# BatsResearch/menghini-neurips23-code

Hardware: AMD Instinct MI355X
Metric: images/sec CLIP ViT-B/16 encode+prompt-step (higher is better)
Workload: dtype f16

## Files before the change

### menghini-neurips23-code_amd/csrc/common.h

```cpp
#pragma once
#include <hip/hip_runtime.h>
#include <stdint.h>
#include <stdio.h>
#include <string.h>

#include "host_common.h"
#include "gemm_plan.h"

typedef _Float16 half_t;
typedef half_t half8 __attribute__((ext_vector_type(8)));
typedef half_t half4 __attribute__((ext_vector_type(4)));
typedef half_t half2v __attribute__((ext_vector_type(2)));
typedef float f32x4 __attribute__((ext_vector_type(4)));

typedef half_t resid_t;

#define AS1 __attribute__((address_space(1)))
#define AS3 __attribute__((address_space(3)))

#define GRIP_CHECK_HIP(expr)                                                                   \
    do {                                                                                       \
        hipError_t _e = (expr);                                                                \
        if (_e != hipSuccess) {                                                                \
            grip_set_error("%s:%d %s -> %s", __FILE__, __LINE__, #expr, hipGetErrorString(_e)); \
// ... 16 lines not shown

__device__ __forceinline__ float wave_sum(float v) {
#define GRIP_DPP_ADD(ctrl) v += __builtin_bit_cast(float, __builtin_amdgcn_update_dpp(0, __builtin_bit_cast(int, v), ctrl, 0xF, 0xF, true))
    GRIP_DPP_ADD(0xB1);
    GRIP_DPP_ADD(0x4E);
    GRIP_DPP_ADD(0x141);
    GRIP_DPP_ADD(0x140);
#undef GRIP_DPP_ADD
    const int b = __builtin_bit_cast(int, v);
    const float r0 = __builtin_bit_cast(float, __builtin_amdgcn_readlane(b, 0)), r1 = __builtin_bit_cast(float, __builtin_amdgcn_readlane(b, 16));
    const float r2 = __builtin_bit_cast(float, __builtin_amdgcn_readlane(b, 32)), r3 = __builtin_bit_cast(float, __builtin_amdgcn_readlane(b, 48));
    return (r0 + r1) + (r2 + r3);
}
__device__ __forceinline__ float row16_sum(float v) {
#define GRIP_DPP_ADD(ctrl) v += __builtin_bit_cast(float, __builtin_amdgcn_update_dpp(0, __builtin_bit_cast(int, v), ctrl, 0xF, 0xF, true))
    GRIP_DPP_ADD(0xB1);
    GRIP_DPP_ADD(0x4E);
    GRIP_DPP_ADD(0x141);
    GRIP_DPP_ADD(0x140);
#undef GRIP_DPP_ADD
    return v;
}

__device__ __forceinline__ f32x4 load4(const float* p, int i) { return ((const f32x4*)p)[i]; }
__device__ __forceinline__ f32x4 load4(const half_t* p, int i) {
    const half4 h = ((const half4*)p)[i];
    return (f32x4){(float)h[0], (float)h[1], (float)h[2], (float)h[3]};
}
__device__ __forceinline__ void store4(float* p, int i, f32x4 v) { ((f32x4*)p)[i] = v; }
__device__ __forceinline__ void store4(half_t* p, int i, f32x4 v) { ((half4*)p)[i] = (half4){(half_t)v[0], (half_t)v[1], (half_t)v[2], (half_t)v[3]}; }
#ifndef GRIP_SPLIT_LO_SCALE
#define GRIP_SPLIT_LO_SCALE 1
#endif
struct SplitRow { half_t* p; };
__device__ __forceinline__ void split_f16x4(f32x4 v, half4& hi, half4& lo) {
#pragma unroll
    for (int e = 0; e < 4; ++e) {
        float x = v[e];
        asm volatile("" : "+v"(x));
        const half_t h = (half_t)x;
        hi[e] = h;
        lo[e] = (half_t)((x - (float)h) * (float)GRIP_SPLIT_LO_SCALE);
    }
}
__device__ __forceinline__ void store4(SplitRow r, int i, f32x4 v) {
    half4 hi, lo;
    split_f16x4(v, hi, lo);
    half_t* o = r.p + (i >> 3) * 64 + (i & 7) * 4;
    *(half4*)o = hi;
    *(half4*)(o + 32) = lo;
}

template <int NV>
__device__ __forceinline__ void ln_normalize(f32x4 (&v)[NV], int lane, int d4, int d, float& mean, float& rstd) {
#pragma clang fp contract(off)
    float s = 0.f;
#pragma unroll
    for (int i = 0; i < NV; ++i)
        if (lane + 64 * i < d4) s += v[i][0] + v[i][1] + v[i][2] + v[i][3];
    mean = wave_sum(s) / (float)d;
    float q = 0.f;
#pragma unroll
    for (int i = 0; i < NV; ++i)
        if (lane + 64 * i < d4) {
            f32x4 c = v[i] - mean;
            q += c[0] * c[0] + c[1] * c[1] + c[2] * c[2] + c[3] * c[3];
// ... 11 lines not shown
    const void* W;
    int M, N, K;
    int variant;
    int64_t m_pad;
    const float* bias;
    const void* resid;
    const void* aux;
    void* out;
    void* out2;
    int ldc;
    float scalar;
    int f32;
    float* stat_part;
    const float* rowstat;
    const float* stat_in;
    int stat_parts;
    const float* colsum;
    int ksplit;
    int64_t split_stride;
    float* coop_scratch;
    int* coop_counter;
    int rot_rows;
    half_t* resid_lo;
    int w_exact;
    int ablate;
};

int launch_gemm(int epi, const GemmArgs& a, hipStream_t s);
int launch_gemm_f32(int epi, const GemmArgs& a, hipStream_t s);
int launch_gemm_split(int epi, const GemmArgs& a, hipStream_t s);
int launch_split_rows(const float* x, void* out, int64_t rows, int K, int64_t ld_in, hipStream_t s, int is_weight = 0, int* overflow_flag = nullptr,
                      int* lo_nonzero_flag = nullptr);
float gemm_split_weight_scale();

int launch_im2col(const void* images, int images_f16, void* out, int out_f32, int B, int R, int patch, int Kpad, hipStream_t s);
int launch_vit_assemble_ln(const float* patch_out, const float* cls, const float* pos, const float* prefix, int P,
                           const float* gamma, const float* beta, void* x, int f32, float* rowstat, int B, int G2, int d, hipStream_t s, half_t* x_lo = nullptr,
                           int per_image = 0);
int launch_vit_deep_insert(const float* deep, void* x, int f32, half_t* x_lo, float* stat_part, float* rowstat, int B, int S, int P, int M, int d, hipStream_t s);
int launch_text_deep_insert(const float* deep, int prefix_classes, void* x, int f32, float* stat_part, float* rowstat, int C, int S, int P, int shared_rows, int M, int d,
                            hipStream_t s);
int launch_ln_stats_finalize(const float* stat_part, int parts, float* rowstat, int M, int d, hipStream_t s);
int launch_ln_fold_weights(const half_t* W, const float* gamma, const float* beta, const float* bias, half_t* Wg, float* colsum, float* bias_out,
                           int N, int K, hipStream_t s);
int launch_layernorm_f16(const void* x, const float* gamma, const float* beta, void* out, int f32, int M, int d, hipStream_t s);
int launch_gather_ln_f16(const void* x, const int32_t* row_index, int row_stride, const float* gamma, const float* beta,
                         void* out, int f32, int n_rows, int d, hipStream_t s);
int launch_text_embed(const int32_t* token_ids, int ld_ids, const float* tok_emb, const float* pos, const float* prefix, int P,
                      int prefix_classes, void* x, int f32, float* rowstat, int C, int T, int d, int vocab, hipStream_t s, int shared_rows = 0);
int launch_transpose(const void* in, void* out, int f32, int rows, int cols, int ld_in, hipStream_t s);

#ifdef __HIPCC__
__device__ __forceinline__ size_t seq_row(int b, int r, int S, int Ps) {
    return r < Ps ? (size_t)r : (size_t)Ps + (size_t)b * (S - Ps) + (r - Ps);
}
#endif

int launch_attention_fwd(const half_t* qkv, half_t* out, int B, int S, int H, int causal, hipStream_t s, int shared_rows = 0);
int launch_attention_row(const half_t* qkv, const half_t* qrows, const int32_t* row_index, half_t* out, int B, int S, int H, int causal, hipStream_t s, int train = 0);
int launch_gather_rows(const half_t* x, const int32_t* row_index, int row_stride, half_t* out, int n_rows, int d, hipStream_t s);
int launch_attention_row_bwd(const half_t* qkv, const half_t* o_rows, const half_t* do_rows, const int32_t* row_index, half_t* dqkv, int B, int S, int H, int causal,
                             hipStream_t s);
int launch_attention_fwd_f32(const float* qkv, float* out, int B, int S, int H, int causal, hipStream_t s, int split_out = 0);
int launch_attention_row_f32(const float* qkv, const float* qrows, const int32_t* row_index, float* out, int B, int S, int H, int causal, hipStream_t s, int split_out = 0);
int launch_gather_rows4(const void* x, const int32_t* row_index, int row_stride, void* out, int n_rows, int d, hipStream_t s);
bool attention_split_supported(int S);
// ... 19 lines not shown
```

### menghini-neurips23-code_amd/csrc/gemm.hip

```cpp
#include <type_traits>

#include "common.h"

#ifndef GRIP_COOP_MODE
#define GRIP_COOP_MODE 2
#endif


#ifndef GRIP_RD0
#define GRIP_RD0 4
#endif
#ifndef GRIP_SETPRIO
#define GRIP_SETPRIO 4
#endif
#ifndef GRIP_SMALL_PRIO
#define GRIP_SMALL_PRIO 0
#endif
#ifndef GRIP_KROT
#define GRIP_KROT 1
#endif

#define BM 128
#define BN 128
#define BK 64
// ... 181 lines not shown
                        if (g.out2) *(half4*)((half_t*)g.out2 + o) = (half4){(half_t)v[0], (half_t)v[1], (half_t)v[2], (half_t)v[3]};
                        v = quick_gelu4(v);
                    }
                    *(half4*)((half_t*)g.out + o) = (half4){(half_t)v[0], (half_t)v[1], (half_t)v[2], (half_t)v[3]};
                } else if constexpr (EPI == EPI_GELUGRAD_F16) {
                    const half4 x = aux[p & 1][it];
                    *(half4*)((half_t*)g.out + o) = (half4){(half_t)(v[0] * quick_gelu_grad((float)x[0])), (half_t)(v[1] * quick_gelu_grad((float)x[1])),
                                                            (half_t)(v[2] * quick_gelu_grad((float)x[2])), (half_t)(v[3] * quick_gelu_grad((float)x[3]))};
                }
            }
        }
        __builtin_amdgcn_wave_barrier();
    }
}

template <int EPI, int ROWFRAGS, int PF = 2, bool PRE = false>
__device__ __forceinline__ void epilogue_rows(const GemmArgs& g, f32x4 (&acc)[ROWFRAGS][4], float* slab, int row0, int col0, int lane,
                                              const float2* pre = nullptr, const f32x4* cb = nullptr) {
    if constexpr (EPI == EPI_BIAS_RESID_STATS) {
        if (g.resid_lo) {
            if (row0 + ROWFRAGS * 16 <= g.M)
                epilogue_rows_impl<EPI, ROWFRAGS, false, PF, PRE, true>(g, acc, slab, row0, col0, lane, pre, cb);
            else
                epilogue_rows_impl<EPI, ROWFRAGS, true, PF, PRE, true>(g, acc, slab, row0, col0, lane, pre, cb);
            return;
        }
    }
    if (row0 + ROWFRAGS * 16 <= g.M)
        epilogue_rows_impl<EPI, ROWFRAGS, false, PF, PRE>(g, acc, slab, row0, col0, lane, pre, cb);
    else
        epilogue_rows_impl<EPI, ROWFRAGS, true, PF, PRE>(g, acc, slab, row0, col0, lane, pre, cb);
}

__device__ __forceinline__ float row8_sum(float v) {
#define GRIP_DPP_ADD(ctrl) v += __builtin_bit_cast(float, __builtin_amdgcn_update_dpp(0, __builtin_bit_cast(int, v), ctrl, 0xF, 0xF, true))
    GRIP_DPP_ADD(0xB1);
    GRIP_DPP_ADD(0x4E);
    GRIP_DPP_ADD(0x141);
#undef GRIP_DPP_ADD
    return v;
}

template <int EPI, bool CHECK, bool PRE, bool HILO = false>
__device__ __forceinline__ void epilogue_rows8_impl(const GemmArgs& g, f32x4 (&acc)[8][4], float* slab, int row0, int col0, int lane, const float2* pre) {
    constexpr bool FOLD = (EPI == EPI_LNFOLD_F16 || EPI == EPI_LNFOLD_GELU_F16);
    constexpr bool RESID = (EPI == EPI_BIAS_RESID_STATS);
    static_assert(FOLD || RESID, "epilogue_rows8: f16-output epilogues of the pool encode only");
    const int frow = lane & 15, fgrp = lane >> 4;
    const int r8 = lane >> 3, c8 = lane & 7;
    const int col = col0 + c8 * 8;
    const int ldc = g.ldc;
    const uint32_t lane_off = (uint32_t)(row0 + r8) * (uint32_t)ldc + (uint32_t)col;
    auto elem_off = [&](int p, int it) -> uint32_t {
        if constexpr (CHECK) {
            int row = row0 + p * 16 + it * 8 + r8;
            row = row < g.M ? row : g.M - 1;
            return (uint32_t)row * (uint32_t)ldc + (uint32_t)col;
        } else {
            return lane_off + (uint32_t)((p * 16 + it * 8) * ldc);
        }
    };
    half8 res[2][2];
    half8 resl[2][HILO ? 2 : 1];
    auto prefetch = [&](int p, int b) {
#pragma unroll
        for (int it = 0; it < 2; ++it) {
// ... 1052 lines not shown
    auto spread = [&]() {
#pragma unroll
        for (int q = 0; q < 12; ++q) {
            __builtin_amdgcn_sched_group_barrier(0x008, 2, 0);
            __builtin_amdgcn_sched_group_barrier(0x100, 1, 0);
        }
    };

    const int nk = g.K / BK;
    auto tile_rot = [&](int tile) {
        int tm, tn;
        tile_coords(tile, tm, tn);
        return k_rot(tn, tiles_n, nk);
    };
    auto ks = [&](int k, int rot) { return k + rot < nk ? k + rot : k + rot - nk; };
    const half_t* src_cur = tile_src(t);
    int rot_cur = tile_rot(t);
    stage(0, src_cur, ks(0, rot_cur));
    stage(1, src_cur, ks(1, rot_cur));
    wait_vmcnt<GI>();
    __builtin_amdgcn_s_barrier();
    int par = 0;
    for (;;) {
        int tm, tn;
        tile_coords(t, tm, tn);
        const int m0 = tm * BMT, n0 = tn * BNT;
        const int t_next = t + per_xcd;
        const bool has_next = t_next < xcount;
        const half_t* src_next = has_next ? tile_src(t_next) : src_cur;
        const int rot_next = has_next ? tile_rot(t_next) : 0;
        if constexpr (EPI == EPI_BIAS_F16 || EPI == EPI_BIAS_GELU_F16 || EPI == EPI_BIAS_RESID || EPI == EPI_BIAS_RESID_STATS) {
#pragma unroll
            for (int j = 0; j < 4; ++j) {
                const f32x4 b = *(const f32x4*)(g.bias + n0 + wc * 64 + (EMODE == 2 ? (lane >> 4) * 16 + j * 4 : j * 16 + (lane >> 4) * 4));
#pragma unroll
                for (int i = 0; i < 8; ++i) acc[i][j] = b;
            }
        } else {
#pragma unroll
            for (int i = 0; i < 8; ++i)
#pragma unroll
                for (int j = 0; j < 4; ++j) acc[i][j] = (f32x4){0.f, 0.f, 0.f, 0.f};
        }
        float2 pre[2];
        if constexpr (EPI == EPI_LNFOLD_F16 || EPI == EPI_LNFOLD_GELU_F16) {
#pragma unroll
            for (int h = 0; h < 2; ++h) {
                int r = m0 + wr * 128 + h * 64 + lane;
                r = r < g.M ? r : g.M - 1;
                pre[h] = ((const float2*)g.rowstat)[r];
            }
        }
        load_frags(0, par, 0);
        for (int kt = 0; kt < nk; ++kt) {
            const int buf = (par + kt) & 1;
            load_frags(1, buf, 1);
            constexpr bool PRIO0 = (GRIP_SETPRIO & 1) && GRIP_SETPRIO < 4;
            constexpr bool PRIO1 = ((GRIP_SETPRIO & 2) && GRIP_SETPRIO < 4) || (GRIP_SETPRIO == 4 && (EPI == EPI_LNFOLD_F16 || EPI == EPI_LNFOLD_GELU_F16));
            if constexpr (PRIO0) __builtin_amdgcn_s_setprio(1);
            mfma_set(0);
            spread();
            if constexpr (PRIO0) __builtin_amdgcn_s_setprio(0);
            asm volatile("s_waitcnt lgkmcnt(0)" ::: "memory");
            wait_vmcnt<0>();
            __builtin_amdgcn_s_barrier();
            if constexpr (PRIO1) __builtin_amdgcn_s_setprio(1);
            if constexpr (SD) {
                const half_t* sp = kt + 2 < nk ? src_cur + (size_t)ks(kt + 2, rot_cur) * BK : (has_next ? src_next + (size_t)ks(kt + 2 - nk, rot_next) * BK : src_cur);
                half_t* dst = lds2 + buf * STAGE + r0 * BK;
                const half_t* st = lds2 + (buf ^ 1) * STAGE;
                constexpr int RD0 = GRIP_RD0;
#pragma unroll
                for (int q = 0; q < 16; ++q) {
#pragma unroll
                    for (int h = 0; h < 2; ++h) {
                        const int mi = (2 * q + h) >> 2, mj = (2 * q + h) & 3;
                        acc[mi][mj] = __builtin_amdgcn_mfma_f32_16x16x32_f16(fb[1][mj], fa[1][mi], acc[mi][mj], 0, 0, 0);
                    }
                    if (q >= RD0 && q < RD0 + 4) fb[0][q - RD0] = *(const half8*)(st + b_off[0] + (q - RD0) * BJ * BK);
                    else if (q >= RD0 + 4 && q < RD0 + 12) fa[0][q - RD0 - 4] = *(const half8*)(st + a_off[0] + (q - RD0 - 4) * 16 * BK);
                    if (q < GI)
                        __builtin_amdgcn_global_load_lds((const AS1 void*)((const char*)(sp + (size_t)q * 8 * K) + lane_off[(q >> 1) & 1]), (AS3 void*)(dst + q * 8 * BK), 16, 0, 0);
                    __builtin_amdgcn_sched_group_barrier(0x008, 2, 0);
                    if (q >= RD0 && q < RD0 + 12) __builtin_amdgcn_sched_group_barrier(0x100, 1, 0);
                    if (q < GI) __builtin_amdgcn_sched_group_barrier(0x010, 1, 0);
                }
            } else {
                if (kt + 2 < nk) stage(buf, src_cur, ks(kt + 2, rot_cur));
                else if (has_next) stage(buf, src_next, ks(kt + 2 - nk, rot_next));
                if (kt + 1 < nk) load_frags(0, buf ^ 1, 0);
                mfma_set(1);
                spread();
            }
            if constexpr (PRIO1) __builtin_amdgcn_s_setprio(0);
        }
        if constexpr (EMODE == 4)
            epilogue_rows8h<EPI, true>(g, acc, (half_t*)slab, m0 + wr * 128, n0 + wc * 64, lane, pre);
        else if constexpr (EMODE == 2)
            epilogue_direct<EPI, (EPI == EPI_LNFOLD_F16 || EPI == EPI_LNFOLD_GELU_F16)>(g, acc, m0 + wr * 128, n0 + wc * 64, lane, pre);
        else if constexpr (EMODE == 1)
            epilogue_rows8<EPI, (EPI == EPI_LNFOLD_F16 || EPI == EPI_LNFOLD_GELU_F16)>(g, acc, slab, m0 + wr * 128, n0 + wc * 64, lane, pre);
        else
            epilogue_rows<EPI, 8, 1, (EPI == EPI_LNFOLD_F16 || EPI == EPI_LNFOLD_GELU_F16)>(g, acc, slab, m0 + wr * 128, n0 + wc * 64, lane, pre);
        if (!has_next) break;
        par = (par + nk) & 1;
        t = t_next;
        src_cur = src_next;
        rot_cur = rot_next;
    }
}

#include <deque>
#include <vector>
namespace {
constexpr int PROF_RING = 4096, PROF_EPIS = 144;
struct ProfRec { int epi; double flops; hipEvent_t a, b; };
bool g_prof = false;
std::deque<ProfRec> g_recs;
std::vector<hipEvent_t> g_pool;
int64_t g_launches[PROF_EPIS];
double g_ms[PROF_EPIS], g_flops[PROF_EPIS];
hipEvent_t prof_event() {
    if (!g_pool.empty()) { hipEvent_t e = g_pool.back(); g_pool.pop_back(); return e; }
    hipEvent_t e = nullptr;
    if (hipEventCreate(&e) != hipSuccess) return nullptr;
    return e;
}
void prof_drain(size_t keep) {
    while (g_recs.size() > keep) {
// ... 129 lines not shown
#ifdef GRIP_ABLATE
    a.ablate = g_ablate;
#endif
    return with_epi(p.epi, [&](auto e) {
        constexpr int E = decltype(e)::value;
        if constexpr (E == EPI_LNFOLD_F16 || E == EPI_LNFOLD_GELU_F16) {
            if (p.sd) return launch_planned<gemm_k64p_kernel<E, (E == EPI_LNFOLD_F16 ? 4 : 2), true>>(p, a, s, p.colgroup);
            switch (p.emode) {
                case 4: return launch_planned<gemm_k64p_kernel<E, 4>>(p, a, s, p.colgroup);
                case 2: return launch_planned<gemm_k64p_kernel<E, 2>>(p, a, s, p.colgroup);
                case 1: return launch_planned<gemm_k64p_kernel<E, 1>>(p, a, s, p.colgroup);
            }
        } else if constexpr (E == EPI_BIAS_RESID_STATS) {
            if (p.sd) return launch_planned<gemm_k64p_kernel<E, 1, true>>(p, a, s, p.colgroup);
            if (p.emode == 1) return launch_planned<gemm_k64p_kernel<E, 1>>(p, a, s, p.colgroup);
        }
        return launch_planned<gemm_k64p_kernel<E>>(p, a, s, p.colgroup);
    });
}

static int gemm_cu_count(int* n_cu) {
    static int n_cu_dev = 0;
    if (!n_cu_dev) {
        int dev = 0;
        GRIP_CHECK_HIP(hipGetDevice(&dev));
        GRIP_CHECK_HIP(hipDeviceGetAttribute(&n_cu_dev, hipDeviceAttributeMultiprocessorCount, dev));
        n_cu_dev &= ~7;
        GRIP_REQUIRE(n_cu_dev >= 8, "gemm: device reports %d CUs", n_cu_dev);
    }
    *n_cu = (grip_cu_budget() > 0 && grip_cu_budget() < n_cu_dev) ? (grip_cu_budget() & ~7) : n_cu_dev;
    return GRIP_OK;
}

static int launch_gemm_impl(int epi, const GemmArgs& a_in, hipStream_t s, int* chosen) {
    GemmShape g{};
    g.epi = epi; g.M = a_in.M; g.N = a_in.N; g.K = a_in.K; g.ldc = a_in.ldc; g.m_pad = a_in.m_pad;
    g.variant = a_in.variant; g.ksplit = a_in.ksplit; g.f32 = a_in.f32; g.rot_rows = a_in.rot_rows;
    g.stat_parts = a_in.stat_parts; g.split_stride = a_in.split_stride;
    g.stat_part = a_in.stat_part; g.stat_in = a_in.stat_in; g.rowstat = a_in.rowstat; g.out2 = a_in.out2; g.coop = a_in.coop_scratch && a_in.coop_counter;
    if (!a_in.f32) {
        const int rc = gemm_cu_count(&g.n_cu);
        if (rc) return rc;
    }
    const GemmPlan p = gemm_plan(g, gemm_tuning());
    if (p.status) {
        grip_set_error("%s", p.msg);
        return p.status;
    }
    *chosen = p.variant;
    GemmArgs a = a_in;
    a.rot_rows = p.rot_rows;
    if (p.finalize_stats) {
        const int rc = launch_ln_stats_finalize(a.stat_in, a.stat_parts, const_cast<float*>(a.rowstat), a.M, a.K, s);
        if (rc) return rc;
        a.stat_parts = 0;
    }
    switch (p.family) {
        case GEMM_SPLIT: return launch_gemm_split(epi, a, s);
        case GEMM_F32: return launch_gemm_f32(epi, a, s);
        case GEMM_TWO_STAGE: return launch_two_stage(p, a, s);
        case GEMM_RING: return launch_ring(p, a, s);
        case GEMM_RINGW: return launch_ringw(p, a, s);
        case GEMM_BIG: return launch_big(p, a, s);
        case GEMM_K64: return launch_k64(p, a, s);
        case GEMM_K64P: return launch_k64p(p, a, s);
    }
// ... 3 lines not shown
```

### menghini-neurips23-code_amd/csrc/gemm_split.hip

```cpp
#include <math.h>

#include "common.h"

#if defined(__HIP_DEVICE_COMPILE__) && !defined(__gfx950__)
#error "gemm_split.hip relies on gfx950 MFMA semantics (unflushed f16 subnormal inputs); build with --offload-arch=gfx950 only"
#endif

#define SPL_BM 256
#define SPL_BN 128
#define SPL_ROWB 128
#define SPL_STAGE_B ((SPL_BM + SPL_BN) * SPL_ROWB)
#define SPL_NST 3
#ifndef SPL_PIPE
#define SPL_PIPE 1
#endif
#define SPL_LO_INV (1.0f / (float)GRIP_SPLIT_LO_SCALE)

__device__ __forceinline__ float quick_gelu_exact_s(float x) { return x * __builtin_amdgcn_rcpf(1.0f + __builtin_amdgcn_exp2f(-1.702f * 1.4426950408889634f * x)); }


#if GRIP_SPLIT_LO_SCALE != 1
template <int EPI>
__global__ __launch_bounds__(512, 2) void gemm_split_kernel(GemmArgs g, int tiles_m, int tiles_n) {
    extern __shared__ __attribute__((aligned(16))) char lds[];

    const int nwg = tiles_m * tiles_n;
    int bid = blockIdx.x;
    {
        const int q = nwg >> 3, r = nwg & 7, xcd = bid & 7, idx = bid >> 3;
        bid = (xcd < r ? xcd * (q + 1) : r * (q + 1) + (xcd - r) * q) + idx;
    }
    const int tm = bid / tiles_n, tn = bid - tm * tiles_n;
    const int m0 = tm * SPL_BM, n0 = tn * SPL_BN;

    const int tid = threadIdx.x;
    const int lane = tid & 63;
    const int wave = __builtin_amdgcn_readfirstlane(tid >> 6);
    const int wr = wave >> 1, wc = wave & 1;

    const int srow = lane >> 3;
    const int schunk = (lane & 7) ^ srow;
    const size_t pitch = (size_t)g.K * 4;
    const char* a_src = (const char*)g.A + (size_t)(m0 + wave * 32) * pitch;
    const char* w_src = (const char*)g.W + (size_t)(n0 + wave * 16) * pitch;
    const uint32_t lane_off = (uint32_t)srow * (uint32_t)pitch + (uint32_t)(schunk * 16);
    auto stage = [&](int slot, int kt) {
        char* abase = lds + slot * SPL_STAGE_B + wave * 32 * SPL_ROWB;
        char* bbase = lds + slot * SPL_STAGE_B + SPL_BM * SPL_ROWB + wave * 16 * SPL_ROWB;
        const char* as = a_src + (size_t)kt * SPL_ROWB;
        const char* ws = w_src + (size_t)kt * SPL_ROWB;
#pragma unroll
// ... 115 lines not shown
#endif
    asm volatile("s_waitcnt vmcnt(0)" ::: "memory");

    constexpr bool HAS_BIAS = (EPI == EPI_BIAS_F16 || EPI == EPI_BIAS_GELU_F16 || EPI == EPI_BIAS_RESID);
    const int row0 = m0 + wr * 64 + frow, col0 = n0 + wc * 64 + fgrp * 4;
#pragma unroll
    for (int j = 0; j < 4; ++j) {
        f32x4 b = {0.f, 0.f, 0.f, 0.f};
        if constexpr (HAS_BIAS) b = *(const f32x4*)(g.bias + col0 + j * 16);
#pragma unroll
        for (int i = 0; i < 4; ++i) {
            const int row = row0 + i * 16;
            if (row >= g.M) continue;
            const int col = col0 + j * 16;
            f32x4 v = acc[i][j] + cor[i][j] * SPL_LO_INV + b;
            if constexpr (EPI == EPI_BIAS_RESID) v += *(const f32x4*)((const float*)g.resid + (size_t)row * g.ldc + col);
            if constexpr (EPI == EPI_BIAS_GELU_F16) {
                v = (f32x4){quick_gelu_exact_s(v[0]), quick_gelu_exact_s(v[1]), quick_gelu_exact_s(v[2]), quick_gelu_exact_s(v[3])};
                store4(SplitRow{(half_t*)g.out + (size_t)row * 2 * g.ldc}, col >> 2, v);
            } else {
                *(f32x4*)((float*)g.out + (size_t)row * g.ldc + col) = v;
            }
        }
    }
}

#endif


#if GRIP_SPLIT_LO_SCALE == 1
#define SP1_BM 256
#define SP1_BN 256
#define SP1_STAGE_B ((SP1_BM + SP1_BN) * SPL_ROWB)
#define SP1_W_SCALE 256.0f
template <int EPI, bool WLO>
__global__ __launch_bounds__(512, 2) void gemm_split1_kernel(GemmArgs g, int tiles_m, int tiles_n) {
    constexpr int FI = 4, FJ = 8;
    extern __shared__ __attribute__((aligned(16))) char lds[];
    const int nwg = tiles_m * tiles_n;
    int bid = blockIdx.x;
    {
        const int q = nwg >> 3, r = nwg & 7, xcd = bid & 7, idx = bid >> 3;
        bid = (xcd < r ? xcd * (q + 1) : r * (q + 1) + (xcd - r) * q) + idx;
    }
    const int tm = bid / tiles_n, tn = bid - tm * tiles_n;
    const int m0 = tm * SP1_BM, n0 = tn * SP1_BN;
    const int tid = threadIdx.x;
    const int lane = tid & 63;
    const int wave = __builtin_amdgcn_readfirstlane(tid >> 6);
    const int wr = wave >> 1, wc = wave & 1;

    const int srow = lane >> 3;
    const int schunk = (lane & 7) ^ srow;
    const size_t pitch = (size_t)g.K * 4;
    const char* a_src = (const char*)g.A + (size_t)(m0 + wave * 32) * pitch;
    const char* w_src = (const char*)g.W + (size_t)(n0 + wave * 32) * pitch;
    const uint32_t lane_off = (uint32_t)srow * (uint32_t)pitch + (uint32_t)(schunk * 16);

    const int frow = lane & 15, fgrp = lane >> 4;
    const int swz_hi = (fgrp ^ (lane & 7)) * 16, swz_lo = ((4 + fgrp) ^ (lane & 7)) * 16;
    const int a_row = (wr * FI * 16 + frow) * SPL_ROWB;
    const int b_row = SP1_BM * SPL_ROWB + (wc * FJ * 16 + frow) * SPL_ROWB;

    f32x4 acc[FI][FJ];
#pragma unroll
    for (int i = 0; i < FI; ++i)
#pragma unroll
        for (int j = 0; j < FJ; ++j) acc[i][j] = (f32x4){0.f, 0.f, 0.f, 0.f};

    const int nk = g.K / 32;
    int ks_stage = (int)(((int64_t)tn * nk) / tiles_n);
    auto next_slice = [&](int k) { return k + 1 == nk ? 0 : k + 1; };
    {
        char* abase = lds + wave * 32 * SPL_ROWB;
        char* bbase = lds + SP1_BM * SPL_ROWB + wave * 32 * SPL_ROWB;
        const char* as = a_src + (size_t)ks_stage * SPL_ROWB;
        const char* ws = w_src + (size_t)ks_stage * SPL_ROWB;
#pragma unroll
        for (int pc = 0; pc < 4; ++pc) {
            __builtin_amdgcn_global_load_lds((const AS1 void*)(as + (size_t)pc * 8 * pitch + lane_off), (AS3 void*)(abase + pc * 8 * SPL_ROWB), 16, 0, 0);
            __builtin_amdgcn_global_load_lds((const AS1 void*)(ws + (size_t)pc * 8 * pitch + lane_off), (AS3 void*)(bbase + pc * 8 * SPL_ROWB), 16, 0, 0);
        }
        ks_stage = next_slice(ks_stage);
    }
    for (int kt = 0; kt < nk; ++kt) {
        asm volatile("s_waitcnt vmcnt(0)" ::: "memory");
        __builtin_amdgcn_s_barrier();
        const char* st = lds + (kt & 1) * SP1_STAGE_B;
        half8 ah[FI], al[FI], wh[FJ], wl[FJ];
        wh[0] = *(const half8*)(st + b_row + swz_hi);
#pragma unroll
        for (int i = 0; i < FI; ++i) ah[i] = *(const half8*)(st + a_row + i * 16 * SPL_ROWB + swz_hi);
#pragma unroll
        for (int j = 1; j < FJ; ++j) wh[j] = *(const half8*)(st + b_row + j * 16 * SPL_ROWB + swz_hi);
        __builtin_amdgcn_sched_barrier(0);
        char* abase = lds + ((kt + 1) & 1) * SP1_STAGE_B + wave * 32 * SPL_ROWB;
        char* bbase = lds + ((kt + 1) & 1) * SP1_STAGE_B + SP1_BM * SPL_ROWB + wave * 32 * SPL_ROWB;
        const char* as = a_src + (size_t)ks_stage * SPL_ROWB;
        const char* ws = w_src + (size_t)ks_stage * SPL_ROWB;
        ks_stage = next_slice(ks_stage);
        constexpr int NQ = WLO ? 96 : 64, PIECE_EVERY = NQ / 8, LO_READS = WLO ? 12 : FI;
#pragma unroll
        for (int q = 0; q < NQ; ++q) {
            const int pass = q >> 5, j = ((q & 31) / FI), i = q % FI;
            if (pass == 0) acc[i][j] = __builtin_amdgcn_mfma_f32_16x16x32_f16(wh[j], ah[i], acc[i][j], 0, 0, 0);
            else if (WLO && pass == 1) acc[i][j] = __builtin_amdgcn_mfma_f32_16x16x32_f16(wl[j], ah[i], acc[i][j], 0, 0, 0);
            else acc[i][j] = __builtin_amdgcn_mfma_f32_16x16x32_f16(wh[j], al[i], acc[i][j], 0, 0, 0);
            if (q < 2 * LO_READS && !(q & 1)) {
                const int r = (q >> 1) + (WLO ? 0 : FJ);
                if (r < FJ) wl[r] = *(const half8*)(st + b_row + r * 16 * SPL_ROWB + swz_lo);
                else al[r - FJ] = *(const half8*)(st + a_row + (r - FJ) * 16 * SPL_ROWB + swz_lo);
                __builtin_amdgcn_sched_barrier(0);
            }
            if (q % PIECE_EVERY == PIECE_EVERY - 1) {
                const int pc = q / PIECE_EVERY;
                if (pc < 4) __builtin_amdgcn_global_load_lds((const AS1 void*)(as + (size_t)pc * 8 * pitch + lane_off), (AS3 void*)(abase + pc * 8 * SPL_ROWB), 16, 0, 0);
                else __builtin_amdgcn_global_load_lds((const AS1 void*)(ws + (size_t)(pc - 4) * 8 * pitch + lane_off), (AS3 void*)(bbase + (pc - 4) * 8 * SPL_ROWB), 16, 0, 0);
                __builtin_amdgcn_sched_barrier(0);
            }
        }
        __builtin_amdgcn_sched_barrier(0);
    }
    asm volatile("s_waitcnt vmcnt(0)" ::: "memory");

    constexpr bool HAS_BIAS = (EPI == EPI_BIAS_F16 || EPI == EPI_BIAS_GELU_F16 || EPI == EPI_BIAS_RESID);
    const int row0 = m0 + wr * FI * 16 + frow, col0 = n0 + wc * FJ * 16 + fgrp * 4;
#pragma unroll
    for (int j = 0; j < FJ; ++j) {
        f32x4 b = {0.f, 0.f, 0.f, 0.f};
        if constexpr (HAS_BIAS) b = *(const f32x4*)(g.bias + col0 + j * 16);
#pragma unroll
        for (int i = 0; i < FI; ++i) {
            const int row = row0 + i * 16;
            if (row >= g.M) continue;
            const int col = col0 + j * 16;
            f32x4 v = acc[i][j] * (1.0f / SP1_W_SCALE) + b;
            if constexpr (EPI == EPI_BIAS_RESID) v += *(const f32x4*)((const float*)g.resid + (size_t)row * g.ldc + col);
            if constexpr (EPI == EPI_BIAS_GELU_F16) {
                v = (f32x4){quick_gelu_exact_s(v[0]), quick_gelu_exact_s(v[1]), quick_gelu_exact_s(v[2]), quick_gelu_exact_s(v[3])};
                store4(SplitRow{(half_t*)g.out + (size_t)row * 2 * g.ldc}, col >> 2, v);
            } else {
                *(f32x4*)((float*)g.out + (size_t)row * g.ldc + col) = v;
            }
        }
    }
}
#endif

__global__ __launch_bounds__(256) void split_rows_kernel(const float* __restrict__ x, half_t* __restrict__ out, int64_t rows, int K, int64_t ld_in, float scale,
                                                         int* __restrict__ overflow, int* __restrict__ lo_nonzero) {
    const int64_t i = (int64_t)blockIdx.x * 256 + threadIdx.x;
    const int k4 = K >> 2;
    if (i >= rows * k4) return;
    const int64_t r = i / k4;
    const int c = (int)(i - r * k4) * 4;
    const f32x4 v = *(const f32x4*)(x + r * ld_in + c) * scale;
    if (overflow) {
        const float m = fmaxf(fmaxf(fabsf(v.x), fabsf(v.y)), fmaxf(fabsf(v.z), fabsf(v.w)));
        if (!(m < 65520.0f)) *overflow = 1;
    }
    if (lo_nonzero) {
        const bool exact = (float)(half_t)v.x == v.x && (float)(half_t)v.y == v.y && (float)(half_t)v.z == v.z && (float)(half_t)v.w == v.w;
        if (!exact) *lo_nonzero = 1;
    }
    store4(SplitRow{out + r * 2 * (int64_t)K}, c >> 2, v);
}

float gemm_split_weight_scale() {
#if GRIP_SPLIT_LO_SCALE == 1
    return SP1_W_SCALE;
#else
    return 1.0f;
#endif
}

int launch_split_rows(const float* x, void* out, int64_t rows, int K, int64_t ld_in, hipStream_t s, int is_weight, int* overflow_flag, int* lo_nonzero_flag) {
    GRIP_REQUIRE(K % 32 == 0 && rows > 0 && ld_in >= K && ld_in % 4 == 0, "split_rows: need K %% 32 == 0 (rows=%lld K=%d ld=%lld)", (long long)rows, K, (long long)ld_in);
    const int64_t n = rows * (K / 4);
    hipLaunchKernelGGL(split_rows_kernel, dim3((unsigned)((n + 255) / 256)), dim3(256), 0, s, x, (half_t*)out, rows, K, ld_in, is_weight ? gemm_split_weight_scale() : 1.0f,
                       overflow_flag, lo_nonzero_flag);
    GRIP_CHECK_HIP(hipGetLastError());
    return GRIP_OK;
}

static int g_last_wlo = -1;
int gemm_split_last_wlo() { return g_last_wlo; }

int launch_gemm_split(int epi, const GemmArgs& a, hipStream_t s) {
    GRIP_REQUIRE(a.K % 64 == 0 && a.M > 0, "gemm_split: need K %% 64 == 0 (M=%d N=%d K=%d)", a.M, a.N, a.K);
    GRIP_REQUIRE(a.ldc % 32 == 0, "gemm_split: ldc %% 32 != 0");
    GRIP_REQUIRE((int64_t)a.K * 4 * 8 < ((int64_t)1 << 31), "gemm_split: K too large for 32-bit lane offsets");
#if GRIP_SPLIT_LO_SCALE == 1
    constexpr int BM = SP1_BM, BN = SP1_BN;
    constexpr size_t lds = (size_t)2 * SP1_STAGE_B;
#define GRIP_SPLIT_KERNEL(E, WLO) gemm_split1_kernel<E, WLO>
#else
    constexpr int BM = SPL_BM, BN = SPL_BN;
    constexpr size_t lds = (size_t)SPL_NST * SPL_STAGE_B;
#define GRIP_SPLIT_KERNEL(E, WLO) gemm_split_kernel<E>
#endif
    GRIP_REQUIRE(a.N % BN == 0, "gemm_split: need N %% %d == 0 (N=%d)", BN, a.N);
    static const bool force_wlo = getenv("GRIP_SPLIT_WLO") && atoi(getenv("GRIP_SPLIT_WLO")) == 1;
    const bool wlo = !a.w_exact || force_wlo;
    g_last_wlo = wlo;
    const int tiles_m = (a.M + BM - 1) / BM, tiles_n = a.N / BN;
    GRIP_REQUIRE(a.m_pad >= (int64_t)tiles_m * BM, "gemm_split: A must be allocated up to the 256-row tile (M=%d m_pad=%lld)", a.M, (long long)a.m_pad);
    dim3 grid(tiles_m * tiles_n), block(512);
#define GRIP_GEMM_LAUNCH(E, WLO)                                                                                            \
    {                                                                                                                       \
        static bool configured = false;                                                                                     \
        if (!configured) {                                                                                                  \
            GRIP_CHECK_HIP(hipFuncSetAttribute((const void*)GRIP_SPLIT_KERNEL(E, WLO), hipFuncAttributeMaxDynamicSharedMemorySize, (int)lds)); \
            configured = true;                                                                                              \
        }                                                                                                                   \
        hipLaunchKernelGGL((GRIP_SPLIT_KERNEL(E, WLO)), grid, block, lds, s, a, tiles_m, tiles_n);                          \
    }
#define GRIP_GEMM_CASE(E)                                                                                                   \
    case E:                                                                                                                 \
        if (wlo) GRIP_GEMM_LAUNCH(E, true) else GRIP_GEMM_LAUNCH(E, false)                                                  \
        break;
    switch (epi) {
        GRIP_GEMM_CASE(EPI_F32)
        GRIP_GEMM_CASE(EPI_BIAS_F16)
        GRIP_GEMM_CASE(EPI_BIAS_GELU_F16)
        GRIP_GEMM_CASE(EPI_BIAS_RESID)
        default: GRIP_REQUIRE(false, "gemm_split: epilogue %d is not part of the split-f16 (inference) path", epi);
    }
#undef GRIP_GEMM_CASE
#undef GRIP_GEMM_LAUNCH
#undef GRIP_SPLIT_KERNEL
    GRIP_CHECK_HIP(hipGetLastError());
    return GRIP_OK;
}
```

### menghini-neurips23-code_amd/csrc/tower.hip

```cpp
#include <stdarg.h>
#include <stdlib.h>

#include <map>
#include <string>
#include <vector>

#include "common.h"

static thread_local char g_err[512] = "";
void grip_set_error(const char* fmt, ...) {
    va_list ap;
    va_start(ap, fmt);
    vsnprintf(g_err, sizeof(g_err), fmt, ap);
    va_end(ap);
}
extern "C" const char* grip_last_error(void) { return g_err; }
extern "C" int grip_abi_version(void) { return GRIP_ABI_VERSION; }

static int g_cu_budget = 0;
int grip_cu_budget() { return g_cu_budget; }
extern "C" int grip_set_cu_budget(int n_cus) {
    GRIP_REQUIRE(n_cus >= 0 && (n_cus == 0 || n_cus >= 8), "set_cu_budget: %d (0 = all, else at least 8)", n_cus);
    g_cu_budget = n_cus;
    return GRIP_OK;
// ... 329 lines not shown
    GRIP_REQUIRE(t, "tower_finalize: null handle");
    hipStream_t s = (hipStream_t)stream;
    const int d = t->D.width;
    int rc;
    const int f = t->f32;
    if (!f)
        for (const LayerW& w : t->L.layer) {
            if ((rc = launch_transpose(t->wop(w.in_w), t->wop(w.in_wT), f, 3 * d, d, d, s))) return rc;
            if ((rc = launch_transpose(t->wop(w.out_w), t->wop(w.out_wT), f, d, d, d, s))) return rc;
            if ((rc = launch_transpose(t->wop(w.fc_w), t->wop(w.fc_wT), f, 4 * d, d, d, s))) return rc;
            if ((rc = launch_transpose(t->wop(w.proj_w), t->wop(w.proj_wT), f, d, 4 * d, 4 * d, s))) return rc;
        }
    if (!f)
        for (const LayerW& w : t->L.layer) {
            float* F = t->w32;
            if ((rc = launch_ln_fold_weights(t->w16 + w.in_w, F + w.ln1_g, F + w.ln1_b, F + w.in_b, t->w16 + w.in_wG, F + w.in_cs, F + w.in_bb, 3 * d, d, s))) return rc;
            if ((rc = launch_ln_fold_weights(t->w16 + w.fc_w, F + w.ln2_g, F + w.ln2_b, F + w.fc_b, t->w16 + w.fc_wG, F + w.fc_cs, F + w.fc_bb, 4 * d, d, s))) return rc;
        }
    if (t->split) {
        int* flag = nullptr;
        GRIP_CHECK_HIP(hipMalloc((void**)&flag, 2 * sizeof(int)));
        hipError_t e = hipMemsetAsync(flag, 0, 2 * sizeof(int), s);
        rc = e == hipSuccess ? GRIP_OK : GRIP_ERR_HIP;
        for (const LayerW& w : t->L.layer) {
            if (rc) break;
            if ((rc = launch_split_rows((const float*)t->wop(w.in_w), t->wop(w.in_wS), 3 * d, d, d, s, 1, flag, flag + 1))) break;
            if ((rc = launch_split_rows((const float*)t->wop(w.out_w), t->wop(w.out_wS), d, d, d, s, 1, flag, flag + 1))) break;
            if ((rc = launch_split_rows((const float*)t->wop(w.fc_w), t->wop(w.fc_wS), 4 * d, d, d, s, 1, flag, flag + 1))) break;
            if ((rc = launch_split_rows((const float*)t->wop(w.proj_w), t->wop(w.proj_wS), d, 4 * d, 4 * d, s, 1, flag, flag + 1))) break;
        }
        int flags[2] = {0, 0};
        if (!rc && (hipMemcpyAsync(flags, flag, 2 * sizeof(int), hipMemcpyDeviceToHost, s) != hipSuccess || hipStreamSynchronize(s) != hipSuccess)) rc = GRIP_ERR_HIP;
        const int over = flags[0];
        t->w_exact = flags[1] == 0;
        (void)hipFree(flag);
        if (rc == GRIP_ERR_HIP) { grip_set_error("tower_finalize: HIP error while splitting the weights"); return rc; }
        if (rc) return rc;
        GRIP_REQUIRE(!over, "tower_finalize: a block weight times %g leaves the f16 range (or is not finite): split-f16 towers (precision 2) need |w| < %g",
                     (double)gemm_split_weight_scale(), 65504.0 / (double)gemm_split_weight_scale());
    }
    if ((rc = launch_transpose(t->wop(t->L.proj), t->wop(t->L.projT), f, d, t->D.embed_dim, t->D.embed_dim, s))) return rc;
    t->finalized = true;
    return GRIP_OK;
}

extern "C" int grip_workspace_bytes(const grip_tower* t, int batch, int n_prefix, int seq_len, int train, size_t* bytes) {
    GRIP_REQUIRE(t && bytes, "workspace_bytes: null pointer");
    try {
        Workspace w;
        int rc = carve(t, batch, n_prefix, train, nullptr, w, seq_len);
        if (rc) return rc;
        *bytes = w.bytes;
        if (t->D.kind == 1 && n_prefix > 0 && !t->f32) {
            Workspace ws;
            rc = carve(t, batch, n_prefix, train, nullptr, ws, seq_len, 1);
            if (rc) return rc;
            if (ws.bytes > *bytes) *bytes = ws.bytes;
        }
        return GRIP_OK;
    } catch (...) { grip_set_error("workspace_bytes: exception"); return GRIP_ERR_ARG; }
}

#define RUN(expr) do { int _rc = (expr); if (_rc) return _rc; } while (0)

static int run_blocks(grip_tower* t, Workspace& w, resid_t* x0, int causal, const int32_t* read_rows, hipStream_t s, resid_t** x_final, bool* compact) {
    const int d = t->D.width, H = t->D.heads, f = t->f32;
    const int gf = t->split ? 2 : f;
    const float* F = t->w32;
    resid_t* x = x0;
    const int parts = d / 64;
// ... 295 lines not shown
    a.A = A; a.W = W; a.M = M; a.N = N; a.K = K; a.m_pad = m_pad; a.bias = bias; a.resid = resid; a.out = out; a.out2 = out2; a.ldc = N;
    a.stat_part = stat_part; a.rowstat = rowstat; a.colsum = colsum;
    return launch_gemm(epi, a, (hipStream_t)stream);
}
extern "C" int grip_debug_gemm_train(int epi, const void* A, const void* W, int M, int N, int K, const float* bias, const void* resid, void* out, void* out2,
                                     float* stat_part, float* rowstat, const float* colsum, const float* stat_in, int stat_parts, int ksplit,
                                     float* coop_scratch, int* coop_counter, int m_pad, void* stream) {
    GemmArgs a{};
    a.rot_rows = 1;
    a.A = A; a.W = W; a.M = M; a.N = N; a.K = K; a.m_pad = m_pad; a.bias = bias; a.resid = resid; a.out = out; a.out2 = out2; a.ldc = N;
    a.stat_part = stat_part; a.rowstat = rowstat; a.colsum = colsum; a.stat_in = stat_in; a.stat_parts = stat_parts;
    a.ksplit = ksplit; a.coop_scratch = coop_scratch; a.coop_counter = coop_counter;
    return launch_gemm(epi, a, (hipStream_t)stream);
}
extern "C" int grip_debug_coop_split(int M, int N, int K) { return gemm_pick_coop_split(M, N, K); }
extern "C" int grip_debug_ln_fold(const void* W, const float* gamma, const float* beta, const float* bias, void* Wg, float* colsum, float* bias_out,
                                  int N, int K, const float* stat_part, int parts, float* rowstat, int M, int d, void* stream) {
    int rc = W ? launch_ln_fold_weights((const half_t*)W, gamma, beta, bias, (half_t*)Wg, colsum, bias_out, N, K, (hipStream_t)stream) : GRIP_OK;
    if (rc || !stat_part) return rc;
    return launch_ln_stats_finalize(stat_part, parts, rowstat, M, d, (hipStream_t)stream);
}
extern "C" int grip_debug_gemm_split(int epi, const float* A, const float* W, int M, int N, int K, const float* bias, const float* resid, void* out,
                                     void* a_split, void* w_split, int m_pad, void* stream) {
    hipStream_t s = (hipStream_t)stream;
    RUN(launch_split_rows(A, a_split, m_pad, K, K, s));
    int* flag = nullptr;
    GRIP_CHECK_HIP(hipMalloc((void**)&flag, sizeof(int)));
    int inexact = 1;
    int rc = hipMemsetAsync(flag, 0, sizeof(int), s) == hipSuccess ? launch_split_rows(W, w_split, N, K, K, s, 1, nullptr, flag) : GRIP_ERR_HIP;
    if (!rc && (hipMemcpyAsync(&inexact, flag, sizeof(int), hipMemcpyDeviceToHost, s) != hipSuccess || hipStreamSynchronize(s) != hipSuccess)) rc = GRIP_ERR_HIP;
    (void)hipFree(flag);
    if (rc) return rc;
    GemmArgs a{};
    a.w_exact = !inexact;
    a.f32 = 2; a.A = a_split; a.W = w_split; a.M = M; a.N = N; a.K = K; a.m_pad = m_pad; a.bias = bias; a.resid = resid; a.out = out; a.ldc = N;
    return launch_gemm(epi, a, s);
}
int gemm_split_last_wlo();
extern "C" int grip_debug_split_last_wlo(void) { return gemm_split_last_wlo(); }
extern "C" int grip_debug_split_rows(const float* x, void* out, int64_t rows, int K, void* stream) {
    return launch_split_rows(x, out, rows, K, K, (hipStream_t)stream);
}
extern "C" int grip_debug_attention_split(const void* qkv, void* out, int B, int S, int H, int causal, int mfma, void* stream) {
    if (mfma) return launch_attention_fwd_split((const float*)qkv, out, B, S, H, causal, (hipStream_t)stream);
    return launch_attention_fwd_f32((const float*)qkv, (float*)out, B, S, H, causal, (hipStream_t)stream, 1);
}
extern "C" int grip_debug_attention_exact(const void* qkv, void* out, int B, int S, int H, int causal, void* stream) {
    return launch_attention_fwd_f32((const float*)qkv, (float*)out, B, S, H, causal, (hipStream_t)stream);
}
extern "C" int grip_debug_attention(const void* qkv, void* out, int B, int S, int H, int causal, void* stream) {
    return launch_attention_fwd((const half_t*)qkv, (half_t*)out, B, S, H, causal, (hipStream_t)stream);
}
extern "C" int grip_debug_attention_shared(const void* qkv, void* out, int B, int S, int H, int shared_rows, void* stream) {
    return launch_attention_fwd((const half_t*)qkv, (half_t*)out, B, S, H, 1, (hipStream_t)stream, shared_rows);
}
extern "C" int grip_debug_attention_row(const void* qkv, const void* qrows, const int32_t* row_index, void* out, int B, int S, int H, int causal, int train,
                                        void* stream) {
    return launch_attention_row((const half_t*)qkv, (const half_t*)qrows, row_index, (half_t*)out, B, S, H, causal, (hipStream_t)stream, train);
}
extern "C" int grip_debug_attention_row_exact(const void* qkv, const void* qrows, const int32_t* row_index, void* out, int B, int S, int H, int causal,
                                              int split_out, void* stream) {
    return launch_attention_row_f32((const float*)qkv, (const float*)qrows, row_index, (float*)out, B, S, H, causal, (hipStream_t)stream, split_out);
}
extern "C" int grip_debug_layernorm(const float* x, const float* gamma, const float* beta, void* out, int M, int d, void* stream) {
    return launch_layernorm_f16_from_f32(x, gamma, beta, (half_t*)out, M, d, (hipStream_t)stream);
}
extern "C" int grip_debug_ln_bwd_add(const void* x, const float* dln, int parts, int64_t part_stride, const float* gamma, float* dx, void* dxh, int M, int d,
                                     void* stream) {
    return launch_ln_bwd_add((const resid_t*)x, dln, parts, part_stride, gamma, dx, (half_t*)dxh, M, d, (hipStream_t)stream);
// ... 252 lines not shown
```

Before: 20320.

## Route exact-weight split GEMMs through the k64p kernel with duplicated hi weights

When the split-f16 weights have no low part (w_exact), the weight hi half is copied into the lo slot at finalize time. The GEMM then runs as an ordinary f16 GEMM over doubled K, so hi*A_hi + hi*A_lo come out as one dot product, using the tuned k64p kernel with a new split epilogue that handles scaling, residual add and GELU. This drops the dedicated two-pass split1 kernel for this case and trades it for the general planned kernel, at the cost of reading the duplicated weights. Whether it runs depends on the workload's precision mode using the split path.

After: 20750 (median of 6 runs). +2.1%, better.

```diff
diff --git a/menghini-neurips23-code_amd/csrc/common.h b/menghini-neurips23-code_amd/csrc/common.h
--- a/menghini-neurips23-code_amd/csrc/common.h
+++ b/menghini-neurips23-code_amd/csrc/common.h
@@ -72,6 +72,8 @@
 #ifndef GRIP_SPLIT_LO_SCALE
 #define GRIP_SPLIT_LO_SCALE 1
 #endif
+#define SP1_W_SCALE 256.0f
+__device__ __forceinline__ float quick_gelu_exact_s(float x) { return x * __builtin_amdgcn_rcpf(1.0f + __builtin_amdgcn_exp2f(-1.702f * 1.4426950408889634f * x)); }
 struct SplitRow { half_t* p; };
 __device__ __forceinline__ void split_f16x4(f32x4 v, half4& hi, half4& lo) {
 #pragma unroll
@@ -149,6 +151,9 @@
 int launch_split_rows(const float* x, void* out, int64_t rows, int K, int64_t ld_in, hipStream_t s, int is_weight = 0, int* overflow_flag = nullptr,
                       int* lo_nonzero_flag = nullptr);
 float gemm_split_weight_scale();
+bool gemm_split_dup_weights();
+int launch_split_dup_weights(const void* src, void* dst, int64_t rows, int K, hipStream_t s);
+int launch_gemm_split_k64p(int epi, const GemmArgs& a, hipStream_t s);
 
 int launch_im2col(const void* images, int images_f16, void* out, int out_f32, int B, int R, int patch, int Kpad, hipStream_t s);
 int launch_vit_assemble_ln(const float* patch_out, const float* cls, const float* pos, const float* prefix, int P,
diff --git a/menghini-neurips23-code_amd/csrc/gemm.hip b/menghini-neurips23-code_amd/csrc/gemm.hip
--- a/menghini-neurips23-code_amd/csrc/gemm.hip
+++ b/menghini-neurips23-code_amd/csrc/gemm.hip
@@ -237,6 +237,65 @@
         epilogue_rows_impl<EPI, ROWFRAGS, true, PF, PRE>(g, acc, slab, row0, col0, lane, pre, cb);
 }
 
+template <int EPI, bool CHECK>
+__device__ __forceinline__ void epilogue_rows_split_impl(const GemmArgs& g, f32x4 (&acc)[8][4], float* slab, int row0, int col0, int lane) {
+    static_assert(EPI == EPI_F32 || EPI == EPI_BIAS_F16 || EPI == EPI_BIAS_GELU_F16 || EPI == EPI_BIAS_RESID, "epilogue_rows_split: the split tier's four epilogues");
+    constexpr bool RESID = (EPI == EPI_BIAS_RESID);
+    const int frow = lane & 15, fgrp = lane >> 4;
+    const int rr = lane >> 4, cc = (lane & 15) * 4;
+    const int col = col0 + cc;
+    const int ldc = g.ldc;
+    const uint32_t lane_off = (uint32_t)(row0 + rr) * (uint32_t)ldc + (uint32_t)col;
+    auto elem_off = [&](int p, int it) -> uint32_t {
+        if constexpr (CHECK) {
+            int row = row0 + p * 16 + it * 4 + rr;
+            row = row < g.M ? row : g.M - 1;
+            return (uint32_t)row * (uint32_t)ldc + (uint32_t)col;
+        } else {
+            return lane_off + (uint32_t)((p * 16 + it * 4) * ldc);
+        }
+    };
+    f32x4 res[2][RESID ? 4 : 1];
+    auto prefetch = [&](int p, int b) {
+#pragma unroll
+        for (int it = 0; it < 4; ++it) res[b][RESID ? it : 0] = *(const f32x4*)((const float*)g.resid + elem_off(p, it));
+    };
+    if constexpr (RESID) prefetch(0, 0);
+#pragma unroll
+    for (int p = 0; p < 8; ++p) {
+#pragma unroll
+        for (int j = 0; j < 4; ++j) *(f32x4*)(slab + slab_off<1>(frow, j * 4 + fgrp)) = acc[p][j] * (1.0f / SP1_W_SCALE);
+        if constexpr (RESID)
+            if (p + 1 < 8) prefetch(p + 1, (p + 1) & 1);
+        __builtin_amdgcn_wave_barrier();
+#pragma unroll
+        for (int it = 0; it < 4; ++it) {
+            const int rl = it * 4 + rr;
+            f32x4 v = *(const f32x4*)(slab + slab_off<1>(rl, lane & 15));
+            const int row = row0 + p * 16 + rl;
+            const uint32_t o = elem_off(p, it);
+            if constexpr (RESID) v += res[p & 1][it];
+            if (!CHECK || row < g.M) {
+                if constexpr (EPI == EPI_BIAS_GELU_F16) {
+                    v = (f32x4){quick_gelu_exact_s(v[0]), quick_gelu_exact_s(v[1]), quick_gelu_exact_s(v[2]), quick_gelu_exact_s(v[3])};
+                    store4(SplitRow{(half_t*)g.out + 2 * (size_t)(o - (uint32_t)col)}, col >> 2, v);
+                } else {
+                    *(f32x4*)((float*)g.out + o) = v;
+                }
+            }
+        }
+        __builtin_amdgcn_wave_barrier();
+    }
+}
+
+template <int EPI>
+__device__ __forceinline__ void epilogue_rows_split(const GemmArgs& g, f32x4 (&acc)[8][4], float* slab, int row0, int col0, int lane) {
+    if (row0 + 128 <= g.M)
+        epilogue_rows_split_impl<EPI, false>(g, acc, slab, row0, col0, lane);
+    else
+        epilogue_rows_split_impl<EPI, true>(g, acc, slab, row0, col0, lane);
+}
+
 __device__ __forceinline__ float row8_sum(float v) {
 #define GRIP_DPP_ADD(ctrl) v += __builtin_bit_cast(float, __builtin_amdgcn_update_dpp(0, __builtin_bit_cast(int, v), ctrl, 0xF, 0xF, true))
     GRIP_DPP_ADD(0xB1);
@@ -1355,7 +1414,8 @@
         if constexpr (EPI == EPI_BIAS_F16 || EPI == EPI_BIAS_GELU_F16 || EPI == EPI_BIAS_RESID || EPI == EPI_BIAS_RESID_STATS) {
 #pragma unroll
             for (int j = 0; j < 4; ++j) {
-                const f32x4 b = *(const f32x4*)(g.bias + n0 + wc * 64 + (EMODE == 2 ? (lane >> 4) * 16 + j * 4 : j * 16 + (lane >> 4) * 4));
+                f32x4 b = *(const f32x4*)(g.bias + n0 + wc * 64 + (EMODE == 2 ? (lane >> 4) * 16 + j * 4 : j * 16 + (lane >> 4) * 4));
+                if constexpr (EMODE == 3) b *= SP1_W_SCALE;
 #pragma unroll
                 for (int i = 0; i < 8; ++i) acc[i][j] = b;
             }
@@ -1417,7 +1477,9 @@
             }
             if constexpr (PRIO1) __builtin_amdgcn_s_setprio(0);
         }
-        if constexpr (EMODE == 4)
+        if constexpr (EMODE == 3)
+            epilogue_rows_split<EPI>(g, acc, slab, m0 + wr * 128, n0 + wc * 64, lane);
+        else if constexpr (EMODE == 4)
             epilogue_rows8h<EPI, true>(g, acc, (half_t*)slab, m0 + wr * 128, n0 + wc * 64, lane, pre);
         else if constexpr (EMODE == 2)
             epilogue_direct<EPI, (EPI == EPI_LNFOLD_F16 || EPI == EPI_LNFOLD_GELU_F16)>(g, acc, m0 + wr * 128, n0 + wc * 64, lane, pre);
@@ -1613,6 +1675,27 @@
     return GRIP_OK;
 }
 
+int launch_gemm_split_k64p(int epi, const GemmArgs& a_in, hipStream_t s) {
+    GemmShape g{};
+    g.epi = epi; g.M = a_in.M; g.N = a_in.N; g.K = 2 * a_in.K; g.ldc = a_in.ldc; g.m_pad = a_in.m_pad; g.variant = 6;
+    const int rc = gemm_cu_count(&g.n_cu);
+    if (rc) return rc;
+    const GemmPlan p = gemm_plan(g, gemm_tuning());
+    if (p.status) {
+        grip_set_error("%s", p.msg);
+        return p.status;
+    }
+    GemmArgs a = a_in;
+    a.K = g.K;
+    switch (epi) {
+        case EPI_F32: return launch_planned<gemm_k64p_kernel<EPI_F32, 3, true>>(p, a, s, p.colgroup);
+        case EPI_BIAS_F16: return launch_planned<gemm_k64p_kernel<EPI_BIAS_F16, 3, true>>(p, a, s, p.colgroup);
+        case EPI_BIAS_GELU_F16: return launch_planned<gemm_k64p_kernel<EPI_BIAS_GELU_F16, 3, true>>(p, a, s, p.colgroup);
+        case EPI_BIAS_RESID: return launch_planned<gemm_k64p_kernel<EPI_BIAS_RESID, 3, true>>(p, a, s, p.colgroup);
+    }
+    GRIP_REQUIRE(false, "gemm_split: epilogue %d is not part of the split-f16 (inference) path", epi);
+}
+
 static int launch_gemm_impl(int epi, const GemmArgs& a_in, hipStream_t s, int* chosen) {
     GemmShape g{};
     g.epi = epi; g.M = a_in.M; g.N = a_in.N; g.K = a_in.K; g.ldc = a_in.ldc; g.m_pad = a_in.m_pad;
diff --git a/menghini-neurips23-code_amd/csrc/gemm_split.hip b/menghini-neurips23-code_amd/csrc/gemm_split.hip
--- a/menghini-neurips23-code_amd/csrc/gemm_split.hip
+++ b/menghini-neurips23-code_amd/csrc/gemm_split.hip
@@ -15,8 +15,6 @@
 #define SPL_PIPE 1
 #endif
 #define SPL_LO_INV (1.0f / (float)GRIP_SPLIT_LO_SCALE)
-
-__device__ __forceinline__ float quick_gelu_exact_s(float x) { return x * __builtin_amdgcn_rcpf(1.0f + __builtin_amdgcn_exp2f(-1.702f * 1.4426950408889634f * x)); }
 
 
 #if GRIP_SPLIT_LO_SCALE != 1
@@ -198,8 +196,7 @@
 #define SP1_BM 256
 #define SP1_BN 256
 #define SP1_STAGE_B ((SP1_BM + SP1_BN) * SPL_ROWB)
-#define SP1_W_SCALE 256.0f
-template <int EPI, bool WLO>
+template <int EPI>
 __global__ __launch_bounds__(512, 2) void gemm_split1_kernel(GemmArgs g, int tiles_m, int tiles_n) {
     constexpr int FI = 4, FJ = 8;
     extern __shared__ __attribute__((aligned(16))) char lds[];
@@ -265,15 +262,15 @@
         const char* as = a_src + (size_t)ks_stage * SPL_ROWB;
         const char* ws = w_src + (size_t)ks_stage * SPL_ROWB;
         ks_stage = next_slice(ks_stage);
-        constexpr int NQ = WLO ? 96 : 64, PIECE_EVERY = NQ / 8, LO_READS = WLO ? 12 : FI;
+        constexpr int NQ = 96, PIECE_EVERY = NQ / 8, LO_READS = 12;
 #pragma unroll
         for (int q = 0; q < NQ; ++q) {
             const int pass = q >> 5, j = ((q & 31) / FI), i = q % FI;
             if (pass == 0) acc[i][j] = __builtin_amdgcn_mfma_f32_16x16x32_f16(wh[j], ah[i], acc[i][j], 0, 0, 0);
-            else if (WLO && pass == 1) acc[i][j] = __builtin_amdgcn_mfma_f32_16x16x32_f16(wl[j], ah[i], acc[i][j], 0, 0, 0);
+            else if (pass == 1) acc[i][j] = __builtin_amdgcn_mfma_f32_16x16x32_f16(wl[j], ah[i], acc[i][j], 0, 0, 0);
             else acc[i][j] = __builtin_amdgcn_mfma_f32_16x16x32_f16(wh[j], al[i], acc[i][j], 0, 0, 0);
             if (q < 2 * LO_READS && !(q & 1)) {
-                const int r = (q >> 1) + (WLO ? 0 : FJ);
+                const int r = q >> 1;
                 if (r < FJ) wl[r] = *(const half8*)(st + b_row + r * 16 * SPL_ROWB + swz_lo);
                 else al[r - FJ] = *(const half8*)(st + a_row + (r - FJ) * 16 * SPL_ROWB + swz_lo);
                 __builtin_amdgcn_sched_barrier(0);
@@ -332,6 +329,32 @@
     store4(SplitRow{out + r * 2 * (int64_t)K}, c >> 2, v);
 }
 
+__global__ __launch_bounds__(256) void split_dup_weights_kernel(const half_t* src, half_t* dst, int64_t n) {
+    const int64_t i = (int64_t)blockIdx.x * 256 + threadIdx.x;
+    if (i >= n) return;
+    const int64_t o = (i >> 2) * 64 + (i & 3) * 8;
+    const half8 v = *(const half8*)(src + o);
+    *(half8*)(dst + o) = v;
+    *(half8*)(dst + o + 32) = v;
+}
+
+int launch_split_dup_weights(const void* src, void* dst, int64_t rows, int K, hipStream_t s) {
+    GRIP_REQUIRE(K % 32 == 0 && rows > 0, "split_dup_weights: need K %% 32 == 0 (rows=%lld K=%d)", (long long)rows, K);
+    const int64_t n = rows * (K / 8);
+    hipLaunchKernelGGL(split_dup_weights_kernel, dim3((unsigned)((n + 255) / 256)), dim3(256), 0, s, (const half_t*)src, (half_t*)dst, n);
+    GRIP_CHECK_HIP(hipGetLastError());
+    return GRIP_OK;
+}
+
+bool gemm_split_dup_weights() {
+#if GRIP_SPLIT_LO_SCALE == 1
+    static const bool force_wlo = getenv("GRIP_SPLIT_WLO") && atoi(getenv("GRIP_SPLIT_WLO")) == 1;
+    return !force_wlo;
+#else
+    return false;
+#endif
+}
+
 float gemm_split_weight_scale() {
 #if GRIP_SPLIT_LO_SCALE == 1
     return SP1_W_SCALE;
@@ -359,31 +382,35 @@
 #if GRIP_SPLIT_LO_SCALE == 1
     constexpr int BM = SP1_BM, BN = SP1_BN;
     constexpr size_t lds = (size_t)2 * SP1_STAGE_B;
-#define GRIP_SPLIT_KERNEL(E, WLO) gemm_split1_kernel<E, WLO>
+#define GRIP_SPLIT_KERNEL(E) gemm_split1_kernel<E>
 #else
     constexpr int BM = SPL_BM, BN = SPL_BN;
     constexpr size_t lds = (size_t)SPL_NST * SPL_STAGE_B;
-#define GRIP_SPLIT_KERNEL(E, WLO) gemm_split_kernel<E>
+#define GRIP_SPLIT_KERNEL(E) gemm_split_kernel<E>
 #endif
     GRIP_REQUIRE(a.N % BN == 0, "gemm_split: need N %% %d == 0 (N=%d)", BN, a.N);
-    static const bool force_wlo = getenv("GRIP_SPLIT_WLO") && atoi(getenv("GRIP_SPLIT_WLO")) == 1;
-    const bool wlo = !a.w_exact || force_wlo;
+    const bool wlo = !a.w_exact;
     g_last_wlo = wlo;
+#if GRIP_SPLIT_LO_SCALE == 1
+    if (!wlo) return launch_gemm_split_k64p(epi, a, s);
+#else
+    GRIP_REQUIRE(wlo, "gemm_split: the scaled-lo build has no two-pass form (GemmArgs::w_exact must be 0)");
+#endif
     const int tiles_m = (a.M + BM - 1) / BM, tiles_n = a.N / BN;
     GRIP_REQUIRE(a.m_pad >= (int64_t)tiles_m * BM, "gemm_split: A must be allocated up to the 256-row tile (M=%d m_pad=%lld)", a.M, (long long)a.m_pad);
     dim3 grid(tiles_m * tiles_n), block(512);
-#define GRIP_GEMM_LAUNCH(E, WLO)                                                                                            \
+#define GRIP_GEMM_LAUNCH(E)                                                                                                 \
     {                                                                                                                       \
         static bool configured = false;                                                                                     \
         if (!configured) {                                                                                                  \
-            GRIP_CHECK_HIP(hipFuncSetAttribute((const void*)GRIP_SPLIT_KERNEL(E, WLO), hipFuncAttributeMaxDynamicSharedMemorySize, (int)lds)); \
+            GRIP_CHECK_HIP(hipFuncSetAttribute((const void*)GRIP_SPLIT_KERNEL(E), hipFuncAttributeMaxDynamicSharedMemorySize, (int)lds)); \
             configured = true;                                                                                              \
         }                                                                                                                   \
-        hipLaunchKernelGGL((GRIP_SPLIT_KERNEL(E, WLO)), grid, block, lds, s, a, tiles_m, tiles_n);                          \
+        hipLaunchKernelGGL((GRIP_SPLIT_KERNEL(E)), grid, block, lds, s, a, tiles_m, tiles_n);                               \
     }
 #define GRIP_GEMM_CASE(E)                                                                                                   \
     case E:                                                                                                                 \
-        if (wlo) GRIP_GEMM_LAUNCH(E, true) else GRIP_GEMM_LAUNCH(E, false)                                                  \
+        GRIP_GEMM_LAUNCH(E)                                                                                                 \
         break;
     switch (epi) {
         GRIP_GEMM_CASE(EPI_F32)
diff --git a/menghini-neurips23-code_amd/csrc/tower.hip b/menghini-neurips23-code_amd/csrc/tower.hip
--- a/menghini-neurips23-code_amd/csrc/tower.hip
+++ b/menghini-neurips23-code_amd/csrc/tower.hip
@@ -385,10 +385,17 @@
         int flags[2] = {0, 0};
         if (!rc && (hipMemcpyAsync(flags, flag, 2 * sizeof(int), hipMemcpyDeviceToHost, s) != hipSuccess || hipStreamSynchronize(s) != hipSuccess)) rc = GRIP_ERR_HIP;
         const int over = flags[0];
-        t->w_exact = flags[1] == 0;
+        t->w_exact = flags[1] == 0 && gemm_split_dup_weights();
         (void)hipFree(flag);
         if (rc == GRIP_ERR_HIP) { grip_set_error("tower_finalize: HIP error while splitting the weights"); return rc; }
         if (rc) return rc;
+        if (t->w_exact)
+            for (const LayerW& w : t->L.layer) {
+                if ((rc = launch_split_dup_weights(t->wop(w.in_wS), t->wop(w.in_wS), 3 * d, d, s))) return rc;
+                if ((rc = launch_split_dup_weights(t->wop(w.out_wS), t->wop(w.out_wS), d, d, s))) return rc;
+                if ((rc = launch_split_dup_weights(t->wop(w.fc_wS), t->wop(w.fc_wS), 4 * d, d, s))) return rc;
+                if ((rc = launch_split_dup_weights(t->wop(w.proj_wS), t->wop(w.proj_wS), d, 4 * d, s))) return rc;
+            }
         GRIP_REQUIRE(!over, "tower_finalize: a block weight times %g leaves the f16 range (or is not finite): split-f16 towers (precision 2) need |w| < %g",
                      (double)gemm_split_weight_scale(), 65504.0 / (double)gemm_split_weight_scale());
     }
@@ -750,9 +757,17 @@
     (void)hipFree(flag);
     if (rc) return rc;
     GemmArgs a{};
-    a.w_exact = !inexact;
+    a.w_exact = !inexact && gemm_split_dup_weights();
     a.f32 = 2; a.A = a_split; a.W = w_split; a.M = M; a.N = N; a.K = K; a.m_pad = m_pad; a.bias = bias; a.resid = resid; a.out = out; a.ldc = N;
-    return launch_gemm(epi, a, s);
+    if (!a.w_exact) return launch_gemm(epi, a, s);
+    void* w_dup = nullptr;
+    GRIP_CHECK_HIP(hipMalloc(&w_dup, (size_t)N * K * 4));
+    a.W = w_dup;
+    rc = launch_split_dup_weights(w_split, w_dup, N, K, s);
+    if (!rc) rc = launch_gemm(epi, a, s);
+    if (hipStreamSynchronize(s) != hipSuccess && !rc) { grip_set_error("debug_gemm_split: HIP error"); rc = GRIP_ERR_HIP; }
+    (void)hipFree(w_dup);
+    return rc;
 }
 int gemm_split_last_wlo();
 extern "C" int grip_debug_split_last_wlo(void) { return gemm_split_last_wlo(); }
```
